# zgojcic/3D_multiview_reg

Measured on AMD Instinct MI355X. Metric: point-cloud pairs/s (feat+match+filter+SVD), 3DMatch 20k-pt, 1/2/4/8 GPU, higher is better.
Workload: dtype f32 (bf16x3 MFMA operands); 1 GPU; one synthetic 3DMatch-scale scene per GPU (configs[2]): 30 fragments x ~20393 voxels (0.025 m) -> FCGF -> rand 5000 samples -> soft feature-NN for all 435 pairs -> OANet (128ch, 500 clusters, 2 blocks) -> weighted Procrustes -> all-gather of (R,t,conf); sampler=rand, fragments_per_gpu=30, pairs_per_gpu=435, samples=5000, voxels_mean=20393, math=f32eq, oanet_point_layout=chunk-major, spconv_presplit_planes=False, spatial_map_order=False, library=2d143fd7778128e4, parallelism=dp1 (one scene per rank, RCCL all-gather of records)

## Files before the change

### 3d_multiview_reg_amd/csrc/knobs.hpp

```cpp
#pragma once

namespace mvr {

constexpr int GPU_CUS = 256;

extern int g_gemm_h;
extern int g_pconv_h;
extern int g_attn_h;
extern int g_spconv_h;
extern int g_feat_nn_fast;

enum ForcePath : int {
  FORCE_FEAT_NN_ONLINE = 0,
  FORCE_GENERIC_GEMM = 1,
  FORCE_UNFUSED_ATTN = 2,
  FORCE_NO_CONV1_FOLD = 3,
  FORCE_POOL_NOSPLIT = 4,
  FORCE_UNPOOL8 = 5,
  FORCE_ROW_LAYOUT = 6,
  FORCE_COUNT = 7
};
extern int g_force[FORCE_COUNT];

}
```

### 3d_multiview_reg_amd/csrc/spconv.hip

```cpp

#include "common.hpp"
#include "knobs.hpp"
#include "mfma_bf16.hpp"
#include "prof.hpp"
#include "sparse.hpp"

namespace mvr {

typedef float floatx16 __attribute__((ext_vector_type(16)));

struct SpArgs {
  const float* in; int64_t ldin; int Cin;
  const int32_t* nbr; int K; int64_t Mout;
  const int32_t* perm;
  const float* W; int Cout;
  const float* bias;
  mvr_bn_p bn; float bn_eps;
  const float* res; int64_t ldres;
  int relu;
  float* out; int64_t ldout;
  int* range; const int* guard; int epoch;
  const uint16_t* inp;
  uint16_t* outp;
};

constexpr int SP_KMAX = 32;
__device__ __attribute__((aligned(16))) float g_sp_zero[4];


#ifndef SP_TRACE
#define SP_TRACE 0
#endif
#if SP_TRACE
__device__ unsigned long long g_sp_trace[8];
#define SPSTAMP(slot)                                                  \
  do {                                                                 \
    unsigned long long t_;                                             \
    __builtin_amdgcn_sched_barrier(0);                                 \
    asm volatile("s_memtime %0\n\ts_waitcnt lgkmcnt(0)" : "=s"(t_));  \
    __builtin_amdgcn_sched_barrier(0);                                 \
    tr[prev_slot] += t_ - t_last;                                      \
    t_last = t_;                                                       \
    prev_slot = (slot);                                                \
  } while (0)
#else
#define SPSTAMP(slot) do {} while (0)
#endif

constexpr int SB_K = 32;
constexpr int SB_BST = 40;
constexpr int SB_CP = 128;
#ifndef SPBX_WBUF
#define SPBX_WBUF 1
#endif
#ifndef SPBX_NS32
#define SPBX_NS32 3
#endif
#ifndef SPBX_NS64
#define SPBX_NS64 3
#endif
#ifndef SPBX_NS128
#define SPBX_NS128 3
#endif
#ifndef SPBX_PS_NS32
#define SPBX_PS_NS32 3
#endif
#ifndef SPBX_PS_NS64
#define SPBX_PS_NS64 3
#endif
#ifndef SPBX_PS_NS128
#define SPBX_PS_NS128 2
#endif

template <int TN, int NS, int H, int PS>
__global__ __launch_bounds__(256, 2) void spconv_bx_kernel(SpArgs a, const uint16_t* __restrict__ wimg, int64_t CoutP,
                                                           const float* __restrict__ isc) {
  using namespace bx;
  constexpr int NPL = planes<H>();
  constexpr float XS = H ? 64.f : 1.f;
  constexpr int TM = 128;
  constexpr int NJ = TN / 32;
  constexpr int BPL = TN * SB_BST;
  constexpr int BG = NPL * BPL * 2 / 16;
  constexpr int GPT = (BG + 255) / 256;
  if (a.guard && *a.guard != a.epoch) return;
  __shared__ __attribute__((aligned(16))) uint16_t Bs[2][NPL * BPL];
  __shared__ int32_t nb[TM][SP_KMAX + 1];
  __shared__ int klist[SP_KMAX];
  __shared__ int orow_s[TM];
  __shared__ unsigned wmask[4];

  const int tid = threadIdx.x, lane = tid & 63, w = tid >> 6;
  const int l32 = lane & 31, h = lane >> 5;
#if SP_TRACE
  unsigned long long tr[8] = {0, 0, 0, 0, 0, 0, 0, 0}, t_last = __builtin_amdgcn_s_memtime();
  int prev_slot = 0;
#endif
  const int gy = (a.Cout + TN - 1) / TN;
  const int64_t t = (int64_t)blockIdx.x;
  const int64_t o0 = (t / gy) * TM;
  const int c0 = (int)(t % gy) * TN;
  const int K = a.K;

  if (tid < TM) {
    const int64_t o = o0 + tid;
    orow_s[tid] = o < a.Mout ? (int)(a.perm ? a.perm[o] : o) : -1;
  }
  __syncthreads();
  {
    constexpr int EMAX = (TM * SP_KMAX + 255) / 256;
    const int dq = 256 / K, dr = 256 - dq * K;
    int row = tid / K, k = tid - row * K;
    int vv[EMAX], ks[EMAX], rs[EMAX];
#pragma unroll
    for (int i = 0; i < EMAX; ++i) {
      ks[i] = k;
      rs[i] = row;
      vv[i] = -1;
      if (row < TM) {
        const int orow = orow_s[row];
        if (orow >= 0) vv[i] = a.nbr ? a.nbr[(int64_t)orow * K + k] : orow;
      }
      row += dq;
      k += dr;
      if (k >= K) {
        k -= K;
        ++row;
      }
    }
    unsigned m = 0;
#pragma unroll
    for (int i = 0; i < EMAX; ++i) {
      if (rs[i] < TM) {
        nb[rs[i]][ks[i]] = vv[i];
        if (vv[i] >= 0) m |= 1u << ks[i];
      }
    }
#pragma unroll
    for (int off = 32; off > 0; off >>= 1) m |= (unsigned)__shfl_xor((int)m, off, 64);
    if (lane == 0) wmask[w] = m;
  }
  __syncthreads();
  const unsigned kmask = wmask[0] | wmask[1] | wmask[2] | wmask[3];
  if (tid < K && ((kmask >> tid) & 1u)) klist[__popc(kmask & ((1u << tid) - 1u))] = tid;
  const int nk = __popc(kmask);
  __syncthreads();

  const int nci = (a.Cin + SB_K - 1) / SB_K;
  const int steps = nk * nci;
  const int row = 32 * w + l32;

  typedef float f32x4 __attribute__((ext_vector_type(4)));
  static_assert(!(PS && H), "pre-split planes are split-bf16");
  struct ASet {
    float4 v[PS ? 1 : 4];
    bf16x8 pv[PS ? 2 : 1][PS ? 3 : 1];
    f32x4 bq[GPT];
  };
  auto load_a = [&](int s, ASet& A) {
    if (s >= steps) s = steps - 1;
    const int k = klist[s / nci];
    const int ci0 = (s % nci) * SB_K;
    const int src = nb[row][k];
    if (PS) {
      const uint16_t* base = a.inp + (int64_t)(src >= 0 ? src : 0) * 3 * a.ldin;
#pragma unroll
      for (int st = 0; st < 2; ++st)
#pragma unroll
        for (int pl = 0; pl < 3; ++pl) {
          const uint16_t* pq = base + pl * a.ldin + ci0 + 16 * st + 8 * h;
          A.pv[st % (PS ? 2 : 1)][pl % (PS ? 3 : 1)] =
              *reinterpret_cast<const bf16x8*>(src >= 0 ? (const void*)pq : (const void*)g_sp_zero);
        }
    } else {
      const float* base = a.in + (int64_t)(src >= 0 ? src : 0) * a.ldin;
#pragma unroll
      for (int q = 0; q < 4; ++q) {
        const int ci = ci0 + 16 * (q >> 1) + 8 * h + 4 * (q & 1);
        const float* pq = src >= 0 ? base + ci : g_sp_zero;
        A.v[q % (PS ? 1 : 4)] = *reinterpret_cast<const float4*>(pq);
      }
    }
    const int cb = s % nci;
    const char* wb = reinterpret_cast<const char*>(wimg) + ((int64_t)(k * nci + cb) * NPL * CoutP + c0) * SB_BST * 2;
#if SPBX_WBUF
    const __amdgpu_buffer_rsrc_t rw = __builtin_amdgcn_make_buffer_rsrc(const_cast<char*>(wb), (short)0, 0x7fffffff,
                                                                        0x00020000);
#pragma unroll
    for (int i = 0; i < GPT; ++i) {
      const int g = min(tid + 256 * i, BG - 1);
      const int pl = g / (TN * 5), wi = g - pl * (TN * 5);
      A.bq[i] = __builtin_bit_cast(f32x4, __builtin_amdgcn_raw_buffer_load_b128(
                                              rw, pl * (int)CoutP * SB_BST * 2 + wi * 16, 0, 0));
    }
#else
#pragma unroll
    for (int i = 0; i < GPT; ++i) {
      const int g = min(tid + 256 * i, BG - 1);
      const int pl = g / (TN * 5), wi = g - pl * (TN * 5);
      A.bq[i] = *reinterpret_cast<const f32x4*>(wb + (int64_t)pl * CoutP * SB_BST * 2 + wi * 16);
    }
#endif
  };
  bool xbad = false;
  float xmx = 0.f;
  auto frag_a = [&](const ASet& A, int st) {
    if (PS) {
      FragT<H> f;
#pragma unroll
      for (int pl = 0; pl < planes<H>(); ++pl)
        f.p[pl] = __builtin_bit_cast(typename FragT<H>::V, A.pv[st % (PS ? 2 : 1)][pl % (PS ? 3 : 1)]);
      return f;
    }
    float v[8];
    const float4 x0 = A.v[(2 * st) % (PS ? 1 : 4)], x1 = A.v[(2 * st + 1) % (PS ? 1 : 4)];
    v[0] = x0.x; v[1] = x0.y; v[2] = x0.z; v[3] = x0.w;
    v[4] = x1.x; v[5] = x1.y; v[6] = x1.z; v[7] = x1.w;
    if (H) {
      float mx = 0.f;
#pragma unroll
      for (int i = 0; i < 8; ++i) {
        v[i] *= XS;
        mx = fmaxf(mx, fabsf(v[i]));
      }
      xbad |= !(mx < F16_RANGE);
      xmx = fmaxf(xmx, mx);
    }
    return split8t<H>(v);
  };
  auto store_b = [&](const ASet& A, int buf) {
    char* dst = reinterpret_cast<char*>(Bs[buf]);
#pragma unroll
    for (int i = 0; i < GPT; ++i) {
      const int g = tid + 256 * i;
      if (g < BG) *reinterpret_cast<f32x4*>(dst + g * 16) = A.bq[i];
    }
  };

  floatx16 acc[NJ];
#pragma unroll
  for (int j = 0; j < NJ; ++j)
#pragma unroll
    for (int r = 0; r < 16; ++r) acc[j][r] = 0.f;

  if (steps > 0) {
    ASet A[NS];
    SPSTAMP(7);
#pragma unroll
    for (int u = 0; u < NS; ++u) load_a(u, A[u]);
    store_b(A[0], 0);
    __syncthreads();
    auto step = [&](int s, ASet& A, const ASet& An) {
      const int cur = s & 1;
      SPSTAMP(1);
      if (s + 1 < steps) store_b(An, cur ^ 1);
      SPSTAMP(2);
      const FragT<H> fa0 = frag_a(A, 0), fa1 = frag_a(A, 1);
      SPSTAMP(3);
      load_a(s + NS, A);
      SPSTAMP(4);
      const uint16_t* Bq = Bs[cur];
#pragma unroll
      for (int st = 0; st < 2; ++st) {
        const FragT<H>& fa = st ? fa1 : fa0;
#pragma unroll
        for (int j = 0; j < NJ; ++j) {
          const uint16_t* bp = Bq + (32 * j + l32) * SB_BST + 16 * st + 8 * h;
          const FragT<H> fb = ld_frag<H>(reinterpret_cast<const char*>(bp), 2 * BPL);
          acc[j] = mma<H>(fa, fb, acc[j]);
        }
      }
      SPSTAMP(5);
      __syncthreads();
    };
    int s = 0;
    for (; s + NS - 1 < steps; s += NS) {
#pragma unroll
      for (int u = 0; u < NS; ++u) step(s + u, A[u], A[(u + 1) % NS]);
    }
#pragma unroll
    for (int u = 0; u < NS - 1; ++u)
      if (s + u < steps) step(s + u, A[u], A[(u + 1) % NS]);
  }

  SPSTAMP(6);
  int orr[16];
#pragma unroll
  for (int r = 0; r < 16; ++r) orr[r] = orow_s[32 * w + (r & 3) + 8 * (r >> 2) + 4 * h];
#pragma unroll
  for (int j = 0; j < NJ; ++j) {
    const int c = c0 + j * 32 + l32;
    if (c >= a.Cout) continue;
    float bsc = 1.f, bsh = 0.f;
    if (a.bn.gamma) {
      bsc = a.bn.gamma[c] / sqrtf(a.bn.var[c] + a.bn_eps);
      bsh = a.bn.beta[c] - a.bn.mean[c] * bsc;
    }
    const float bias = a.bias ? a.bias[c] : 0.f;
    const float is = H ? isc[c] : 1.f;
    float rv[16];
#pragma unroll
    for (int r = 0; r < 16; ++r) rv[r] = a.res && orr[r] >= 0 ? a.res[(int64_t)orr[r] * a.ldres + c] : 0.f;
#pragma unroll
    for (int r = 0; r < 16; ++r) {
      if (orr[r] < 0) continue;
      float v = (H ? acc[j][r] * is : acc[j][r]) + bias;
      v = fmaf(v, bsc, bsh);
      if (a.res) v += rv[r];
      if (a.relu) v = fmaxf(v, 0.f);
      a.out[(int64_t)orr[r] * a.ldout + c] = v;
      if (a.outp) bx::store_planes(a.outp + (int64_t)orr[r] * 3 * a.ldout + c, a.ldout, v);
    }
  }
  if (H && __any(xbad || (xmx > 0.f && xmx < 0.125f)) && lane == 0) atomicExch(a.range, a.epoch);
#if SP_TRACE
  SPSTAMP(0);
  if (lane == 0)
// ... 40 lines not shown
  uint16_t* row = img + ((kb * 3) * CoutP + c) * SB_BST + 8 * q;
  *reinterpret_cast<bf16x8*>(row) = f.h;
  *reinterpret_cast<bf16x8*>(row + CoutP * SB_BST) = f.m;
  *reinterpret_cast<bf16x8*>(row + 2 * CoutP * SB_BST) = f.l;
  const float sc = wsc[c];
#pragma unroll
  for (int i = 0; i < 8; ++i) v[i] *= sc;
  const FragT<1> g = split8t<1>(v);
  uint16_t* row16 = img16 + ((kb * 2) * CoutP + c) * SB_BST + 8 * q;
  *reinterpret_cast<f16x8*>(row16) = g.p[0];
  *reinterpret_cast<f16x8*>(row16 + CoutP * SB_BST) = g.p[1];
}

#ifndef SPCONV_MATH_DEFAULT
#define SPCONV_MATH_DEFAULT 0
#endif
int g_spconv_h = SPCONV_MATH_DEFAULT;

}

using namespace mvr;

static int64_t sp_coutp(int Cout) { return ((int64_t)Cout + SB_CP - 1) / SB_CP * SB_CP; }

static size_t sp_bf16_bytes(int K, int Cin, int Cout) {
  return (size_t)K * ((Cin + SB_K - 1) / SB_K) * 3 * sp_coutp(Cout) * SB_BST * 2;
}
static size_t sp_f16_bytes(int K, int Cin, int Cout) { return sp_bf16_bytes(K, Cin, Cout) / 3 * 2; }

extern "C" size_t mvr_spconv_wimage_bytes(int K, int Cin, int Cout) {
  if (K <= 0 || Cin <= 0 || Cout <= 0) return 0;
  return sp_bf16_bytes(K, Cin, Cout) + sp_f16_bytes(K, Cin, Cout) + 2 * sp_coutp(Cout) * sizeof(float);
}

extern "C" int mvr_spconv_wimage(const float* W, int K, int Cin, int Cout, void* img, size_t bytes, hipStream_t s) {
  if (!W || !img || K <= 0 || K > SP_KMAX || Cin <= 0 || Cout <= 0 || bytes < mvr_spconv_wimage_bytes(K, Cin, Cout) ||
      (reinterpret_cast<uintptr_t>(img) & 15))
    return MVR_EINVAL;
  const int nci = (Cin + SB_K - 1) / SB_K;
  const int64_t CoutP = sp_coutp(Cout);
  const int64_t total = (int64_t)K * nci * CoutP * 4;
  char* base = reinterpret_cast<char*>(img);
  uint16_t* img16 = reinterpret_cast<uint16_t*>(base + sp_bf16_bytes(K, Cin, Cout));
  float* wsc = reinterpret_cast<float*>(base + sp_bf16_bytes(K, Cin, Cout) + sp_f16_bytes(K, Cin, Cout));
  hipLaunchKernelGGL(spconv_wscale_kernel, dim3((unsigned)((CoutP * 64 + 255) / 256)), dim3(256), 0, s, W, K, Cin, Cout,
                     CoutP, wsc, wsc + CoutP);
  MVR_CHECK_LAUNCH();
  hipLaunchKernelGGL(spconv_wimage_kernel, dim3((unsigned)((total + 255) / 256)), dim3(256), 0, s, W, K, Cin, Cout, nci,
                     CoutP, reinterpret_cast<uint16_t*>(img), img16, wsc);
  MVR_CHECK_LAUNCH();
  return MVR_OK;
}

extern "C" int mvr_spconv_x(const float* in, int64_t ldin, int Cin, const int32_t* nbr, const int32_t* perm, int K,
                            int64_t Mout, const float* W, int Cout, const float* bias, mvr_bn_p bn, float bn_eps,
                            const float* res, int64_t ldres, int relu, float* out, int64_t ldout, const void* wimg,
                            int32_t* range_flag, const uint16_t* in_planes, uint16_t* out_planes, hipStream_t s) {
  if (Cin <= 0 || Cout <= 0 || K <= 0 || K > SP_KMAX || Mout < 0) return MVR_EINVAL;
  if (Mout == 0) return MVR_OK;
  if (!in || !W || !out || !wimg) return MVR_EINVAL;
  if ((in_planes && ((ldin & 7) || (reinterpret_cast<uintptr_t>(in_planes) & 15))) ||
      (out_planes && (reinterpret_cast<uintptr_t>(out_planes) & 1)))
    return MVR_EINVAL;
  if (reinterpret_cast<uintptr_t>(wimg) & 15) return MVR_EINVAL;
  if (!nbr && K != 1) return MVR_EINVAL;
  if ((Cin % SB_K) || (Cout & 3) || (ldin & 3) || (reinterpret_cast<uintptr_t>(in) & 15) ||
      (reinterpret_cast<uintptr_t>(W) & 15))
    return MVR_EINVAL;
  SpArgs a{in, ldin, Cin, nbr, K, Mout, perm, W, Cout, bias, bn, bn_eps, res, ldres, relu, out, ldout,
           nullptr, nullptr, 0, in_planes, out_planes};
  ProfScope prof(PK_SPCONV, 2.0 * Mout * (double)K * Cin * Cout,
                 (double)Mout * (Cin + Cout) * 4.0 + (nbr ? (double)Mout * K * 4.0 : 0.0) + 4.0 * K * Cin * Cout, s);
  const char* base = reinterpret_cast<const char*>(wimg);
  const uint16_t* wi = reinterpret_cast<const uint16_t*>(wimg);
  const uint16_t* wi16 = reinterpret_cast<const uint16_t*>(base + sp_bf16_bytes(K, Cin, Cout));
  const int64_t CoutP = sp_coutp(Cout);
  const float* isc = reinterpret_cast<const float*>(base + sp_bf16_bytes(K, Cin, Cout) + sp_f16_bytes(K, Cin, Cout)) +
                     CoutP;
  const unsigned gx = (unsigned)((Mout + 127) / 128);
  const bool h1 = g_spconv_h && range_flag && Cout > 64 && res != out;
  if (h1) {
    if (hipMemsetAsync(range_flag, 0, sizeof(int32_t), s) != hipSuccess) return MVR_ELAUNCH;
    a.range = range_flag;
    a.epoch = 1;
  }
#define MVR_SPL(TN_, NS_, PNS_, GY)                                                                             \
  do {                                                                                                         \
    if (h1) {                                                                                                  \
      hipLaunchKernelGGL((spconv_bx_kernel<TN_, NS_, 1, 0>), dim3(gx * (GY)), dim3(256), 0, s, a, wi16, CoutP, isc); \
      MVR_CHECK_LAUNCH();                                                                                      \
      a.guard = a.range;                                                                                       \
      a.range = nullptr;                                                                                       \
    }                                                                                                          \
    if (in_planes)                                                                                             \
      hipLaunchKernelGGL((spconv_bx_kernel<TN_, PNS_, 0, 1>), dim3(gx * (GY)), dim3(256), 0, s, a, wi, CoutP, isc); \
    else                                                                                                       \
      hipLaunchKernelGGL((spconv_bx_kernel<TN_, NS_, 0, 0>), dim3(gx * (GY)), dim3(256), 0, s, a, wi, CoutP, isc); \
  } while (0)
  if (Cout <= 32)
    MVR_SPL(32, SPBX_NS32, SPBX_PS_NS32, 1);
  else if (Cout <= 64)
    MVR_SPL(64, SPBX_NS64, SPBX_PS_NS64, (Cout + 63) / 64);
  else
    MVR_SPL(128, SPBX_NS128, SPBX_PS_NS128, (Cout + 127) / 128);
#undef MVR_SPL
  MVR_CHECK_LAUNCH();
  return MVR_OK;
}

extern "C" int mvr_spconv(const float* in, int64_t ldin, int Cin, const int32_t* nbr, const int32_t* perm, int K,
                          int64_t Mout, const float* W, int Cout, const float* bias, mvr_bn_p bn, float bn_eps,
                          const float* res, int64_t ldres, int relu, float* out, int64_t ldout, const void* wimg,
                          int32_t* range_flag, hipStream_t s) {
  return mvr_spconv_x(in, ldin, Cin, nbr, perm, K, Mout, W, Cout, bias, bn, bn_eps, res, ldres, relu, out, ldout, wimg,
                      range_flag, nullptr, nullptr, s);
}

#if SP_TRACE
extern "C" int mvr_spconv_trace(unsigned long long* out, int reset) {
  if (hipMemcpyFromSymbol(out, HIP_SYMBOL(mvr::g_sp_trace), sizeof(unsigned long long) * 8) != hipSuccess) return -1;
  if (reset) {
    unsigned long long z[8] = {0, 0, 0, 0, 0, 0, 0, 0};
    if (hipMemcpyToSymbol(HIP_SYMBOL(mvr::g_sp_trace), z, sizeof(z)) != hipSuccess) return -1;
  }
  return 0;
}
#endif
```

### 3d_multiview_reg_amd/lib/_native.py

```python
import ctypes
import os

import torch

_PKG = os.path.dirname(os.path.dirname(os.path.abspath(__file__)))
LIB_PATH = os.environ.get("MVR_LIB") or os.path.join(_PKG, "libmvreg_hip.so")
_lib = None

c_i64 = ctypes.c_int64
c_int = ctypes.c_int
c_float = ctypes.c_float
c_vp = ctypes.c_void_p
c_size = ctypes.c_size_t


class ConvP(ctypes.Structure):
    _fields_ = [("weight", c_vp), ("bias", c_vp)]


class BnP(ctypes.Structure):
    _fields_ = [("gamma", c_vp), ("beta", c_vp), ("mean", c_vp), ("var", c_vp)]


class PointCNP(ctypes.Structure):
# ... 72 lines not shown
    "mvr_radius_index_bytes": (c_size, [c_i64]),
    "mvr_radius_index_build": (c_int, [c_vp, c_vp, c_int, c_i64, ctypes.c_double, c_vp, c_size, c_vp]),
    "mvr_radius_overlap_count": (c_int, [c_vp, c_size, c_vp, c_vp, c_int, c_i64, c_vp, c_vp, c_int, c_i64,
                                         ctypes.c_double, c_vp, c_vp]),
    "mvr_icp_refine": (c_int, [c_vp, c_size, c_vp, c_vp, c_int, c_i64, ctypes.c_double, c_vp, c_vp, c_int,
                               ctypes.c_double, c_int, ctypes.c_double, ctypes.c_double, c_vp, c_vp, c_vp, c_vp, c_vp,
                               c_vp, c_vp, c_vp]),
    "mvr_estimate_normals": (c_int, [c_vp, c_size, c_vp, c_vp, c_int, c_i64, ctypes.c_double, ctypes.c_double, c_vp,
                                     c_vp, c_vp, c_vp]),
    "mvr_icp_refine_plane": (c_int, [c_vp, c_size, c_vp, c_vp, c_vp, c_int, c_i64, ctypes.c_double, c_vp, c_vp, c_int,
                                     ctypes.c_double, c_int, ctypes.c_double, ctypes.c_double, c_vp, c_vp, c_vp, c_vp,
                                     c_vp, c_vp, c_vp, c_vp]),
    "mvr_icp_refine_generalized": (c_int, [c_vp, c_size, c_vp, c_vp, c_vp, c_int, c_i64, ctypes.c_double, c_vp, c_vp,
                                           c_int, ctypes.c_double, ctypes.c_double, c_int, ctypes.c_double,
                                           ctypes.c_double, c_vp, c_vp, c_vp, c_vp, c_vp, c_vp, c_vp, c_vp]),
    "mvr_pair_information": (c_int, [c_vp, c_size, c_vp, c_vp, c_int, c_i64, ctypes.c_double, c_vp, c_vp, c_int,
                                     ctypes.c_double, c_vp, c_vp, c_vp, c_vp, c_vp]),
    "mvr_compute_fpfh_workspace_bytes": (c_size, [c_i64]),
    "mvr_compute_fpfh": (c_int, [c_vp, c_size, c_vp, c_vp, c_vp, c_int, c_i64, ctypes.c_double, ctypes.c_double, c_vp,
                                 c_vp, c_vp, c_size, c_vp]),
    "mvr_feat_match": (c_int, [c_vp, c_int, c_vp, c_int, c_i64, c_vp, c_vp, c_int, c_i64, c_i64, c_vp, c_vp, c_vp]),
    "mvr_posegraph_workspace_bytes": (c_size, [c_int, c_int, c_int]),
    "mvr_posegraph_optimize": (c_int, [c_vp, c_vp, c_vp, c_vp, c_vp, c_i64, c_vp, c_vp, c_int, c_int, c_int, c_int,
                                       c_vp, c_vp, c_int, ctypes.c_double, ctypes.c_double, ctypes.c_double, c_vp,
                                       c_vp, c_i64, c_vp, c_vp, c_vp, c_vp, c_vp, c_vp, c_size, c_vp]),
    "mvr_fuse_scene_workspace_bytes": (c_size, [c_i64]),
    "mvr_fuse_scene": (c_int, [c_vp, c_vp, c_vp, c_int, c_i64, c_vp, c_vp, ctypes.c_double, c_vp, c_size, c_vp, c_vp,
                               c_vp, c_vp, c_vp, c_vp]),
    "mvr_hash_table_bytes": (c_size, [c_i64]),
    "mvr_voxelize_workspace_bytes": (c_size, [c_i64]),
    "mvr_voxelize_hint_workspace_bytes": (c_size, [c_i64, c_i64]),
    "mvr_voxelize_hint": (c_int, [c_vp, c_vp, c_int, c_i64, ctypes.c_double, c_i64, c_vp, c_size, c_vp, c_vp, c_vp,
                                  c_vp]),
    "mvr_voxelize": (c_int, [c_vp, c_vp, c_int, c_i64, ctypes.c_double, c_vp, c_size, c_vp, c_vp, c_vp, c_vp]),
    "mvr_voxelize_f64": (c_int, [c_vp, c_vp, c_int, c_i64, ctypes.c_double, c_vp, c_size, c_vp, c_vp, c_vp, c_vp]),
    "mvr_coords_downsample_workspace_bytes": (c_size, [c_i64]),
    "mvr_coords_downsample": (c_int, [c_vp, c_i64, c_int, c_int, c_vp, c_size, c_vp, c_vp, c_vp]),
    "mvr_hash_build": (c_int, [c_vp, c_i64, c_vp, c_size, c_vp]),
    "mvr_hash_build_lattice": (c_int, [c_vp, c_i64, c_int, c_vp, c_size, c_vp]),
    "mvr_kernel_map": (c_int, [c_vp, c_i64, c_vp, c_size, c_int, c_int, c_int, c_vp, c_vp]),
    "mvr_kernel_map_x": (c_int, [c_vp, c_i64, c_vp, c_size, c_int, c_int, c_int, c_vp, c_vp, c_vp]),
    "mvr_kernel_map_sym": (c_int, [c_vp, c_i64, c_vp, c_size, c_int, c_vp, c_vp]),
    "mvr_kernel_map_transpose": (c_int, [c_vp, c_i64, c_int, c_vp, c_i64, c_vp]),
    "mvr_kernel_map_order_bytes": (c_size, [c_i64]),
    "mvr_kernel_map_order": (c_int, [c_vp, c_vp, c_int, c_i64, c_int, c_vp, c_vp, c_size, c_vp]),
    "mvr_kernel_map_orders_bytes": (c_size, [c_i64]),
    "mvr_kernel_map_orders": (c_int, [c_int, c_vp, c_vp, c_vp, c_vp, c_int, c_vp, c_vp, c_size, c_vp]),
    "mvr_radix_sort_pairs_bytes": (c_size, [c_i64]),
    "mvr_radix_sort_pairs": (c_int, [c_vp, c_vp, c_i64, c_int, c_vp, c_vp, c_size, c_vp]),
    "mvr_spconv": (c_int, [c_vp, c_i64, c_int, c_vp, c_vp, c_int, c_i64, c_vp, c_int, c_vp, BnP, c_float, c_vp, c_i64,
                           c_int, c_vp, c_i64, c_vp, c_vp, c_vp]),
    "mvr_spconv_x": (c_int, [c_vp, c_i64, c_int, c_vp, c_vp, c_int, c_i64, c_vp, c_int, c_vp, BnP, c_float, c_vp,
                             c_i64, c_int, c_vp, c_i64, c_vp, c_vp, c_vp, c_vp, c_vp]),
    "mvr_spconv_c1_x": (c_int, [c_vp, c_i64, c_vp, c_i64, c_size, c_vp, c_int, c_int, c_vp, c_int, BnP, c_float,
                                c_int, c_vp, c_i64, c_vp, c_vp]),
    "mvr_spconv_wimage_bytes": (c_size, [c_int, c_int, c_int]),
    "mvr_spconv_wimage": (c_int, [c_vp, c_int, c_int, c_int, c_vp, c_size, c_vp]),
    "mvr_brick_map_bytes": (c_size, [c_i64]),
    "mvr_brick_map_build": (c_int, [c_vp, c_i64, c_vp, c_size, c_vp]),
    "mvr_brick_map_build_stride": (c_int, [c_vp, c_i64, c_int, c_vp, c_size, c_vp]),
    "mvr_spconv_c1": (c_int, [c_vp, c_i64, c_vp, c_i64, c_size, c_vp, c_int, c_int, c_vp, c_int, BnP, c_float, c_int,
                              c_vp, c_i64, c_vp]),
    "mvr_l2norm_rows": (c_int, [c_vp, c_i64, c_int, c_i64, c_vp]),
    "mvr_prof_set": (c_int, [c_int]),
    "mvr_prof_mask": (c_int, [ctypes.c_uint]),
    "mvr_prof_seq": (c_int, [c_vp, c_vp, c_int]),
    "mvr_prof_get": (c_int, [c_int, ctypes.POINTER(ctypes.c_double), ctypes.POINTER(ctypes.c_longlong),
                             ctypes.POINTER(ctypes.c_double), ctypes.POINTER(ctypes.c_double)]),
    "mvr_oan_last_layout": (c_int, []),
    "mvr_source_hash": (c_int, [ctypes.c_char_p, c_size]),
    "mvr_xs_to_channels": (c_int, [c_vp, c_i64, c_i64, c_int, c_int, c_int, c_vp, c_i64, c_i64, c_vp]),
}

EXPORTS = tuple(_SIGS)


def lib():
    global _lib
    if _lib is None:
        if not os.path.exists(LIB_PATH):
            raise RuntimeError("libmvreg_hip.so not found at %s — run __graft_entry__.build() "
                               "(there is no CPU fallback for the HIP path)" % LIB_PATH)
        L = ctypes.CDLL(LIB_PATH)
        for name, (res, args) in _SIGS.items():
            f = getattr(L, name)
            f.restype = res
            f.argtypes = args
        _lib = L
    return _lib


_hip_ok = False


def require_hip(t=None):
    global _hip_ok
    if not _hip_ok:
        if not torch.cuda.is_available():
            raise RuntimeError("mvreg HIP path: no HIP device available (no CPU fallback)")
        _hip_ok = True
    if t is not None and t.device.type != "cuda":
        raise RuntimeError("mvreg HIP path: tensor on %s, expected a HIP device" % t.device)


def stream():
    return c_vp(torch.cuda.current_stream().cuda_stream)
# ... 1 lines not shown

def ptr(t):
    if t is None:
        return None
    return c_vp(t.data_ptr())


def check(rc, name):
    if rc != 0:
        raise RuntimeError("%s failed with code %d" % (name, rc))


def source_hash():
    buf = ctypes.create_string_buffer(128)
    check(lib().mvr_source_hash(buf, len(buf)), "mvr_source_hash")
    return buf.value.decode()


PROF_KINDS = {"conv_pts": 0, "embed": 1, "pool": 2, "unpool": 3, "oafilter": 4, "small": 5, "procrustes": 6,
              "feat_nn": 7, "spconv": 8, "sparse_misc": 9, "pointcn": 10}
RANSAC_CHECKED_PROF = {"check": 11, "scan": 12, "eval": 13, "select": 14}


def prof_set(on):
    check(lib().mvr_prof_set(int(on)), "mvr_prof_set")


def prof_mask(kinds=None):
    m = 0xFFFFFFFF if kinds is None else sum(1 << (PROF_KINDS[k] if isinstance(k, str) else int(k)) for k in kinds)
    check(lib().mvr_prof_mask(m), "mvr_prof_mask")


def prof_seq():
    import numpy as np
    L = lib()
    n = L.mvr_prof_seq(None, None, 0)
    k = np.zeros(max(n, 1), np.int32)
    b = np.zeros(max(n, 1), np.float64)
    L.mvr_prof_seq(k.ctypes.data, b.ctypes.data, n)
    names = {v: s for s, v in PROF_KINDS.items()}
    return [(names.get(int(k[i]), str(int(k[i]))), float(b[i])) for i in range(n)]


def prof_get(kind):
    ms, n, fl, by = ctypes.c_double(), ctypes.c_longlong(), ctypes.c_double(), ctypes.c_double()
    k = PROF_KINDS[kind] if isinstance(kind, str) else int(kind)
    check(lib().mvr_prof_get(k, ctypes.byref(ms), ctypes.byref(n), ctypes.byref(fl), ctypes.byref(by)),
          "mvr_prof_get")
    return ms.value, n.value, fl.value, by.value


MATH_KERNELS = "pconv_math,attn_math,spconv_math,gemm_f16,feat_nn"
FORCE = {"feat_nn_online": 0, "generic_gemm": 1, "unfused_attn": 2, "no_conv1_fold": 3, "pool_nosplit": 4,
         "unpool8": 5, "row_layout": 6}


def math_state():
    L = lib()
    m = L.mvr_set_math(0)
    L.mvr_set_math(m)
    return m


def set_math(mode):
    L = lib()
    L.mvr_set_math({"f32eq": 0, "split16": 1}[mode])
    m = math_state()
    dtype = "f32 (bf16x3 MFMA operands)" if not m else "mixed: split-fp16 (22-bit) operands in " + MATH_KERNELS
    return {"mode": "split16" if m else "f32eq", "dtype": dtype, "knobs": {"split16": m}}


class force:

    def __init__(self, what, value=1):
        self.what, self.value = FORCE[what], int(value)

    def __enter__(self):
        self.prev = lib().mvr_debug_force(self.what, self.value)
        return self

    def __exit__(self, *a):
        lib().mvr_debug_force(self.what, self.prev)


_ws_cache = {}
_flag_cache = {}


def flag_word(device=None):
    idx = (device.index if device is not None and device.index is not None else torch.cuda.current_device())
    key = (idx, torch.cuda.current_stream(idx).cuda_stream)
    buf = _flag_cache.get(key)
    if buf is None:
        buf = torch.zeros(64, dtype=torch.int32, device=torch.device("cuda", idx))
        _flag_cache[key] = buf
    return buf


def workspace(nbytes, device):
    idx = device.index if device.index is not None else torch.cuda.current_device()
    key = (idx, torch.cuda.current_stream(idx).cuda_stream)
    buf = _ws_cache.get(key)
    if buf is None or buf.numel() < nbytes:
        buf = torch.empty(max(int(nbytes), 1), dtype=torch.uint8, device=device)
        _ws_cache[key] = buf
    if _WS_POISON:
        buf[:int(nbytes)].fill_(0x7F)
# ... 5 lines not shown
```

### 3d_multiview_reg_amd/lib/descriptor/fcgf.py

```python
import os

import torch
import torch.nn as nn

from lib import _native as N
from lib.sparse import SparseTensor


CONV1_BRICKS = os.environ.get("MVR_CONV1_BRICKS", "1") == "1"
PRESPLIT = os.environ.get("MVR_SPCONV_PRESPLIT", "0") == "1"


def _planes(M, ld, dev):
    return torch.empty(M, 3, ld, dtype=torch.int16, device=dev) if PRESPLIT else None


class _MEConv(nn.Module):

    def __init__(self, cin, cout, ksize, has_bias=False):
        super().__init__()
        self.kernel_size = ksize
        self.kernel = nn.Parameter(torch.empty(ksize ** 3, cin, cout))
        nn.init.kaiming_normal_(self.kernel.data.view(-1, cout), nonlinearity="relu")
        self.bias = nn.Parameter(torch.zeros(1, cout)) if has_bias else None
# ... 30 lines not shown
        self.norm2 = _MENorm(planes, bn_momentum)


def _bn(norm):
    if norm is None:
        return N.BnP(None, None, None, None), 1e-5
    b = norm.bn
    return N.BnP(b.weight.data_ptr(), b.bias.data_ptr(), b.running_mean.data_ptr(), b.running_var.data_ptr()), b.eps


class FCGFNet(nn.Module):
    NORM_TYPE = "BN"
    BLOCK_NORM_TYPE = "BN"
    CHANNELS = [None, 32, 64, 128, 256]
    TR_CHANNELS = [None, 64, 64, 64, 128]

    def __init__(self, in_channels=1, out_channels=32, bn_momentum=0.05, normalize_feature=True,
                 conv1_kernel_size=7, D=3):
        super().__init__()
        C, T = self.CHANNELS, self.TR_CHANNELS
        self.D = D
        self.normalize_feature = normalize_feature
        self.conv1_kernel_size = conv1_kernel_size
        self.conv1 = _MEConv(in_channels, C[1], conv1_kernel_size)
        self.norm1 = _MENorm(C[1], bn_momentum)
        self.block1 = BasicBlockBN(C[1], C[1], bn_momentum)
        self.conv2 = _MEConv(C[1], C[2], 3)
        self.norm2 = _MENorm(C[2], bn_momentum)
        self.block2 = BasicBlockBN(C[2], C[2], bn_momentum)
        self.conv3 = _MEConv(C[2], C[3], 3)
        self.norm3 = _MENorm(C[3], bn_momentum)
        self.block3 = BasicBlockBN(C[3], C[3], bn_momentum)
        self.conv4 = _MEConv(C[3], C[4], 3)
        self.norm4 = _MENorm(C[4], bn_momentum)
        self.block4 = BasicBlockBN(C[4], C[4], bn_momentum)
        self.conv4_tr = _MEConv(C[4], T[4], 3)
        self.norm4_tr = _MENorm(T[4], bn_momentum)
        self.block4_tr = BasicBlockBN(T[4], T[4], bn_momentum)
        self.conv3_tr = _MEConv(C[3] + T[4], T[3], 3)
        self.norm3_tr = _MENorm(T[3], bn_momentum)
        self.block3_tr = BasicBlockBN(T[3], T[3], bn_momentum)
        self.conv2_tr = _MEConv(C[2] + T[3], T[2], 3)
        self.norm2_tr = _MENorm(T[2], bn_momentum)
        self.block2_tr = BasicBlockBN(T[2], T[2], bn_momentum)
        self.conv1_tr = _MEConv(C[1] + T[2], T[1], 1)
        self.final = _MEConv(T[1], out_channels, 1, has_bias=True)

    def _conv(self, x, ldx, conv, km, M, out, ldout, norm=None, res=None, ldres=0, relu=False, bias=None, xp=None,
              outp=None):
        bnp, eps = _bn(norm)
        K, cin, cout = conv.kernel.shape
        nbr, perm = km if km is not None else (None, None)
        wimg = conv.wimage()
        N.check(N.lib().mvr_spconv_x(N.ptr(x), ldx, cin, N.ptr(nbr), N.ptr(perm), K, M, N.ptr(conv.kernel), cout,
                                     N.ptr(bias), bnp, eps, N.ptr(res), ldres, int(relu), N.ptr(out), ldout,
                                     N.ptr(wimg), N.ptr(N.flag_word(x.device)), N.ptr(xp), N.ptr(outp), N.stream()),
                "mvr_spconv_x")
        return out

    def _block(self, blk, x, ldx, km, M, out, ldout, xp=None, outp=None):
        c = blk.conv1.kernel.shape[2]
        t = torch.empty(M, c, device=x.device)
        tp = _planes(M, c, x.device)
        self._conv(x, ldx, blk.conv1, km, M, t, c, blk.norm1, relu=True, xp=xp, outp=tp)
        self._conv(t, c, blk.conv2, km, M, out, ldout, blk.norm2, res=x, ldres=ldx, relu=True, xp=tp, outp=outp)
        return out

    def forward(self, x):
        N.require_hip()
        f32 = torch.float32
        if not all(t.is_cuda and t.dtype is f32 and t.is_contiguous()
                   for t in (*self.parameters(), *self.buffers()) if t.dtype.is_floating_point):
            raise RuntimeError("FCGFNet parameters must be contiguous float32 on a HIP device")
        if self.training:
            raise NotImplementedError("FCGFNet on the HIP path runs in eval mode (BatchNorm running statistics)")
        cm = x.coords_man
        cm.prepare_orders()

        def km(kind, s):
            return cm.kernel_map(kind, s), cm.kernel_map_order(kind, s)
        dev = x.F.device
        C, T = self.CHANNELS, self.TR_CHANNELS
        M = [cm.coords_at(s).shape[0] for s in (1, 2, 4, 8)]
        L = N.lib()
        feat = x.F.float().contiguous()
        if feat.shape[1] != 1:
            raise NotImplementedError("conv1 kernel supports in_channels=1 (all reference configs)")
        s1 = torch.empty(M[0], C[1], device=dev)
        bnp, eps = _bn(self.norm1)
        bricks = cm.brick_map(1)
        oc = None if (self.conv1_kernel_size == 7 and CONV1_BRICKS) else N.ptr(cm.coords_at(1))
        s1p = _planes(M[0], C[1], dev) if oc is None else None
        N.check(L.mvr_spconv_c1_x(oc, M[0], N.ptr(bricks), M[0], bricks.numel(), N.ptr(feat),
                                  self.conv1_kernel_size, 1, N.ptr(self.conv1.kernel), C[1], bnp, eps, 0, N.ptr(s1),
                                  C[1], N.ptr(s1p), N.stream()), "mvr_spconv_c1_x")
        cat1 = torch.empty(M[0], T[2] + C[1], device=dev)
        cat2 = torch.empty(M[1], T[3] + C[2], device=dev)
        cat3 = torch.empty(M[2], T[4] + C[3], device=dev)
        w1, w2, w3 = cat1.shape[1], cat2.shape[1], cat3.shape[1]
        cat1p, cat2p, cat3p = (_planes(M[i], w, dev) for i, w in ((0, w1), (1, w2), (2, w3)))
        skip1, skip2, skip3 = cat1[:, T[2]:], cat2[:, T[3]:], cat3[:, T[4]:]

        def sl(p, c0):
            return p[:, :, c0:] if p is not None else None
        skip1p, skip2p, skip3p = sl(cat1p, T[2]), sl(cat2p, T[3]), sl(cat3p, T[4])
        self._block(self.block1, s1, C[1], km("s1", 1), M[0], skip1, w1, s1p, skip1p)
        t2 = torch.empty(M[1], C[2], device=dev)
        t2p = _planes(M[1], C[2], dev)
        self._conv(skip1, w1, self.conv2, km("down", 1), M[1], t2, C[2], self.norm2, xp=skip1p, outp=t2p)
        self._block(self.block2, t2, C[2], km("s1", 2), M[1], skip2, w2, t2p, skip2p)
# ... 32 lines not shown
```

### include/mvreg.h

```cpp
#ifndef MVREG_H
#define MVREG_H
#include <stddef.h>
#include <stdint.h>

#ifdef __cplusplus
extern "C" {
#endif

typedef struct ihipStream_t* mvr_stream_t;

#define MVR_OK 0
#define MVR_EINVAL -1
#define MVR_ELAUNCH -2

int mvr_procrustes(const float* x1, const float* x2, int64_t x_pstride, int64_t x_nstride, float* w,
                   int64_t w_pstride, const int32_t* guard_pos, float* w_copy, int64_t wc_pstride, int P, int N,
                   int normalize, float eps, float* R, float* t, float* res, int64_t res_pstride, float* res_copy,
                   int64_t rc_pstride, int32_t* status, int guard_group, mvr_stream_t stream);
int mvr_procrustes_f64(const double* x1, const double* x2, int64_t x_pstride, int64_t x_nstride, double* w,
                       int64_t w_pstride, const int32_t* guard_pos, double* w_copy, int64_t wc_pstride, int P, int N,
                       int normalize, double eps, double* R, double* t, double* res, int64_t res_pstride,
                       double* res_copy, int64_t rc_pstride, int32_t* status, int guard_group,
                       mvr_stream_t stream);

// ... 172 lines not shown
int mvr_feat_nn_gumbel(const float* Fq, int64_t fq_fstride, const float* Ft, int64_t ft_fstride, const float* Xq,
                       int64_t xq_fstride, const float* Xt, int64_t xt_fstride, const int64_t* pairs, int P, int Nq,
                       int Mt, int C, float inv_tau, int hard, uint64_t seed, float* out, int64_t out_pstride,
                       int64_t out_nstride, int32_t* idx_out, mvr_stream_t stream);

int mvr_feat_knn2(const float* Fq, int64_t fq_fstride, const float* Ft, int64_t ft_fstride, const int64_t* pairs,
                  int P, int Nq, int Mt, int C, int32_t* idx2_out, double* dist2_out, mvr_stream_t stream);

int mvr_gather_rows(const float* src, int C, const int64_t* idx, int n, float* dst, mvr_stream_t stream);

size_t mvr_hash_table_bytes(int64_t M);
size_t mvr_voxelize_workspace_bytes(int64_t n);
int mvr_voxelize(const float* xyz, const int64_t* frag_off, int B, int64_t n, double voxel, void* workspace,
                 size_t workspace_bytes, int32_t* coords_out, int64_t* sel_out, int64_t* counts_out,
                 mvr_stream_t stream);
int mvr_voxelize_f64(const double* xyz, const int64_t* frag_off, int B, int64_t n, double voxel, void* workspace,
                     size_t workspace_bytes, int32_t* coords_out, int64_t* sel_out, int64_t* counts_out,
                     mvr_stream_t stream);
size_t mvr_voxelize_hint_workspace_bytes(int64_t n, int64_t distinct_hint);
int mvr_voxelize_hint(const float* xyz, const int64_t* frag_off, int B, int64_t n, double voxel,
                      int64_t distinct_hint, void* ws, size_t ws_bytes, int32_t* coords_out, int64_t* sel_out,
                      int64_t* counts_out, mvr_stream_t stream);
size_t mvr_coords_downsample_workspace_bytes(int64_t M);
int mvr_coords_downsample(const int32_t* coords, int64_t M, int B, int stride_out, void* workspace,
                          size_t workspace_bytes, int32_t* coords_out, int64_t* counts_out, mvr_stream_t stream);
int mvr_hash_build(const int32_t* coords, int64_t M, void* table, size_t table_bytes, mvr_stream_t stream);
int mvr_hash_build_lattice(const int32_t* coords, int64_t M, int stride, void* table, size_t table_bytes,
                           mvr_stream_t stream);
int mvr_kernel_map(const int32_t* out_coords, int64_t Mout, const void* in_table, size_t in_table_bytes, int ksize,
                   int step, int transposed, int32_t* nbr, mvr_stream_t stream);
int mvr_kernel_map_x(const int32_t* out_coords, int64_t Mout, const void* in_table, size_t in_table_bytes, int ksize,
                     int step, int transposed, int32_t* nbr, const int32_t* row_order, mvr_stream_t stream);
int mvr_kernel_map_sym(const int32_t* coords, int64_t M, const void* table, size_t table_bytes, int step, int32_t* nbr,
                       mvr_stream_t stream);
int mvr_kernel_map_transpose(const int32_t* src, int64_t Ms, int K, int32_t* dst, int64_t Md, mvr_stream_t stream);
size_t mvr_kernel_map_order_bytes(int64_t Mout);
int mvr_kernel_map_order(const int32_t* nbr, const int32_t* out_coords, int step, int64_t Mout, int K, int32_t* perm,
                         void* workspace, size_t workspace_bytes, mvr_stream_t stream);
size_t mvr_kernel_map_orders_bytes(int64_t total);
int mvr_kernel_map_orders(int n_maps, const int32_t* const* nbr, const int32_t* const* out_coords, const int* steps,
                          const int64_t* Mo, int K, int32_t* perm_out, void* workspace, size_t workspace_bytes,
                          mvr_stream_t stream);
size_t mvr_radix_sort_pairs_bytes(int64_t n);
int mvr_radix_sort_pairs(const uint64_t* keys, const int32_t* vals, int64_t n, int bits, int32_t* vals_out,
                         void* workspace, size_t workspace_bytes, mvr_stream_t stream);
int mvr_spconv(const float* in, int64_t ldin, int Cin, const int32_t* nbr, const int32_t* perm, int K, int64_t Mout,
               const float* W, int Cout, const float* bias, mvr_bn_p bn, float bn_eps, const float* res,
               int64_t ldres, int relu, float* out, int64_t ldout, const void* wimg, int32_t* range_flag,
               mvr_stream_t stream);
int mvr_spconv_x(const float* in, int64_t ldin, int Cin, const int32_t* nbr, const int32_t* perm, int K, int64_t Mout,
                 const float* W, int Cout, const float* bias, mvr_bn_p bn, float bn_eps, const float* res,
                 int64_t ldres, int relu, float* out, int64_t ldout, const void* wimg, int32_t* range_flag,
                 const uint16_t* in_planes, uint16_t* out_planes, mvr_stream_t stream);
size_t mvr_spconv_wimage_bytes(int K, int Cin, int Cout);
int mvr_spconv_wimage(const float* W, int K, int Cin, int Cout, void* img, size_t bytes, mvr_stream_t stream);
size_t mvr_brick_map_bytes(int64_t M);
int mvr_brick_map_build(const int32_t* coords, int64_t M, void* workspace, size_t workspace_bytes,
                        mvr_stream_t stream);
int mvr_brick_map_build_stride(const int32_t* coords, int64_t M, int stride, void* workspace, size_t workspace_bytes,
                               mvr_stream_t stream);
int mvr_spconv_c1(const int32_t* out_coords, int64_t Mout, const void* in_bricks, int64_t Min, size_t in_bricks_bytes,
                  const float* feat, int ksize, int step, const float* W, int Cout, mvr_bn_p bn, float bn_eps,
                  int relu, float* out, int64_t ldout, mvr_stream_t stream);
int mvr_spconv_c1_x(const int32_t* out_coords, int64_t Mout, const void* in_bricks, int64_t Min,
                    size_t in_bricks_bytes, const float* feat, int ksize, int step, const float* W, int Cout,
                    mvr_bn_p bn, float bn_eps, int relu, float* out, int64_t ldout, uint16_t* out_planes,
                    mvr_stream_t stream);
int mvr_l2norm_rows(float* x, int64_t M, int C, int64_t ld, mvr_stream_t stream);

int mvr_sample_rand_mt19937(uint32_t* key, int32_t* pos, const int64_t* counts, int B, int tgt, int64_t* out,
                            int64_t* ws);

int mvr_prof_set(int on);
int mvr_prof_mask(unsigned mask);
int mvr_prof_get(int kind, double* ms, long long* launches, double* flops, double* bytes);
int mvr_prof_seq(int* kinds, double* bytes, int cap);
int mvr_source_hash(char* buf, size_t cap);

#ifdef __cplusplus
}
#endif
#endif
```

Before: 10620 pairs/s.

## Use 32-bit buffer-resource loads with precomputed byte offsets in sparse conv

Adds a sparse-conv kernel variant that stores each neighbour index as a premultiplied byte offset, with INT_MIN marking a missing neighbour. Input and weight-image gathers go through AMD buffer resource loads, which return zero for out-of-range offsets, so the 64-bit address arithmetic and the per-step zero-pointer select are no longer needed. The active-kernel list is walked with an incremental bitmask iterator, which drops the klist shared-memory build and one block barrier. The variant is chosen only when the input row count is passed and the tensor sizes fit in 31-bit offsets. It adds a new entry point and a force flag that falls back to the old path.

```diff
diff --git a/3d_multiview_reg_amd/csrc/knobs.hpp b/3d_multiview_reg_amd/csrc/knobs.hpp
--- a/3d_multiview_reg_amd/csrc/knobs.hpp
+++ b/3d_multiview_reg_amd/csrc/knobs.hpp
@@ -18,7 +18,8 @@
   FORCE_POOL_NOSPLIT = 4,
   FORCE_UNPOOL8 = 5,
   FORCE_ROW_LAYOUT = 6,
-  FORCE_COUNT = 7
+  FORCE_SPCONV_ADDR64 = 7,
+  FORCE_COUNT = 8
 };
 extern int g_force[FORCE_COUNT];
 
diff --git a/3d_multiview_reg_amd/csrc/spconv.hip b/3d_multiview_reg_amd/csrc/spconv.hip
--- a/3d_multiview_reg_amd/csrc/spconv.hip
+++ b/3d_multiview_reg_amd/csrc/spconv.hip
@@ -1,3 +1,5 @@
+
+#include <climits>
 
 #include "common.hpp"
 #include "knobs.hpp"
@@ -22,6 +24,7 @@
   int* range; const int* guard; int epoch;
   const uint16_t* inp;
   uint16_t* outp;
+  uint32_t in_bytes;
 };
 
 constexpr int SP_KMAX = 32;
@@ -53,6 +56,9 @@
 #ifndef SPBX_WBUF
 #define SPBX_WBUF 1
 #endif
+#ifndef SPBX_GBUF
+#define SPBX_GBUF 1
+#endif
 #ifndef SPBX_NS32
 #define SPBX_NS32 3
 #endif
@@ -72,7 +78,7 @@
 #define SPBX_PS_NS128 2
 #endif
 
-template <int TN, int NS, int H, int PS>
+template <int TN, int NS, int H, int PS, int BO>
 __global__ __launch_bounds__(256, 2) void spconv_bx_kernel(SpArgs a, const uint16_t* __restrict__ wimg, int64_t CoutP,
                                                            const float* __restrict__ isc) {
   using namespace bx;
@@ -128,10 +134,12 @@
         ++row;
       }
     }
+    const int rowb = (int)a.ldin * (PS ? 6 : 4);
     unsigned m = 0;
 #pragma unroll
     for (int i = 0; i < EMAX; ++i) {
       if (rs[i] < TM) {
+        if (BO) vv[i] = vv[i] >= 0 ? vv[i] * rowb : INT_MIN;
         nb[rs[i]][ks[i]] = vv[i];
         if (vv[i] >= 0) m |= 1u << ks[i];
       }
@@ -141,10 +149,14 @@
     if (lane == 0) wmask[w] = m;
   }
   __syncthreads();
-  const unsigned kmask = wmask[0] | wmask[1] | wmask[2] | wmask[3];
-  if (tid < K && ((kmask >> tid) & 1u)) klist[__popc(kmask & ((1u << tid) - 1u))] = tid;
+  unsigned kmask = wmask[0] | wmask[1] | wmask[2] | wmask[3];
+  if (BO) {
+    kmask = (unsigned)__builtin_amdgcn_readfirstlane((int)kmask);
+  } else {
+    if (tid < K && ((kmask >> tid) & 1u)) klist[__popc(kmask & ((1u << tid) - 1u))] = tid;
+  }
   const int nk = __popc(kmask);
-  __syncthreads();
+  if (!BO) __syncthreads();
 
   const int nci = (a.Cin + SB_K - 1) / SB_K;
   const int steps = nk * nci;
@@ -157,7 +169,52 @@
     bf16x8 pv[PS ? 2 : 1][PS ? 3 : 1];
     f32x4 bq[GPT];
   };
-  auto load_a = [&](int s, ASet& A) {
+  unsigned lrem = kmask;
+  int lk = kmask ? __builtin_ctz(kmask) : 0, lcb = 0;
+  const int hb = (PS ? 16 : 32) * h;
+  const int wstep = NPL * (int)CoutP * SB_BST * 2;
+  const void* gbase = PS ? (const void*)a.inp : (const void*)a.in;
+  const __amdgpu_buffer_rsrc_t rin =
+      __builtin_amdgcn_make_buffer_rsrc(const_cast<void*>(gbase), (short)0, (int)a.in_bytes, 0x00020000);
+  const __amdgpu_buffer_rsrc_t rwi = __builtin_amdgcn_make_buffer_rsrc(
+      const_cast<char*>(reinterpret_cast<const char*>(wimg)) + (int64_t)c0 * SB_BST * 2, (short)0, 0x7fffffff,
+      0x00020000);
+  int woff[GPT];
+#pragma unroll
+  for (int i = 0; i < GPT; ++i) {
+    const int g = min(tid + 256 * i, BG - 1);
+    const int pl = g / (TN * 5), wi = g - pl * (TN * 5);
+    woff[i] = pl * (int)CoutP * SB_BST * 2 + wi * 16;
+  }
+  auto load_a = [&](int s, ASet& A, const FragT<H>* fa = nullptr) {
+    if (BO) {
+      int off = nb[row][lk];
+      if (!PS && fa) asm volatile("" : "+v"(off) : "v"(fa[0].p[NPL - 1]), "v"(fa[1].p[NPL - 1]));
+      const int vo = off + hb;
+      if (PS) {
+#pragma unroll
+        for (int st = 0; st < 2; ++st)
+#pragma unroll
+          for (int pl = 0; pl < 3; ++pl)
+            A.pv[st % (PS ? 2 : 1)][pl % (PS ? 3 : 1)] = __builtin_bit_cast(
+                bf16x8, __builtin_amdgcn_raw_buffer_load_b128(rin, vo + 32 * st, pl * (int)a.ldin * 2 + lcb * SB_K * 2, 0));
+      } else {
+#pragma unroll
+        for (int q = 0; q < 4; ++q)
+          A.v[q % (PS ? 1 : 4)] = __builtin_bit_cast(
+              float4, __builtin_amdgcn_raw_buffer_load_b128(rin, vo + 64 * (q >> 1) + 16 * (q & 1), lcb * SB_K * 4, 0));
+      }
+      const int ws = (lk * nci + lcb) * wstep;
+#pragma unroll
+      for (int i = 0; i < GPT; ++i)
+        A.bq[i] = __builtin_bit_cast(f32x4, __builtin_amdgcn_raw_buffer_load_b128(rwi, woff[i], ws, 0));
+      const unsigned nrem = lrem & (lrem - 1);
+      const bool inblk = lcb + 1 < nci, next = !inblk && nrem != 0;
+      lcb = inblk ? lcb + 1 : (next ? 0 : lcb);
+      lrem = next ? nrem : lrem;
+      lk = next ? __builtin_ctz(nrem) : lk;
+      return;
+    }
     if (s >= steps) s = steps - 1;
     const int k = klist[s / nci];
     const int ci0 = (s % nci) * SB_K;
@@ -255,14 +312,14 @@
       SPSTAMP(1);
       if (s + 1 < steps) store_b(An, cur ^ 1);
       SPSTAMP(2);
-      const FragT<H> fa0 = frag_a(A, 0), fa1 = frag_a(A, 1);
+      const FragT<H> faq[2] = {frag_a(A, 0), frag_a(A, 1)};
       SPSTAMP(3);
-      load_a(s + NS, A);
+      load_a(s + NS, A, faq);
       SPSTAMP(4);
       const uint16_t* Bq = Bs[cur];
 #pragma unroll
       for (int st = 0; st < 2; ++st) {
-        const FragT<H>& fa = st ? fa1 : fa0;
+        const FragT<H>& fa = faq[st];
 #pragma unroll
         for (int j = 0; j < NJ; ++j) {
           const uint16_t* bp = Bq + (32 * j + l32) * SB_BST + 16 * st + 8 * h;
@@ -409,10 +466,11 @@
   return MVR_OK;
 }
 
-extern "C" int mvr_spconv_x(const float* in, int64_t ldin, int Cin, const int32_t* nbr, const int32_t* perm, int K,
+extern "C" int mvr_spconv_n(const float* in, int64_t ldin, int Cin, const int32_t* nbr, const int32_t* perm, int K,
                             int64_t Mout, const float* W, int Cout, const float* bias, mvr_bn_p bn, float bn_eps,
                             const float* res, int64_t ldres, int relu, float* out, int64_t ldout, const void* wimg,
-                            int32_t* range_flag, const uint16_t* in_planes, uint16_t* out_planes, hipStream_t s) {
+                            int32_t* range_flag, const uint16_t* in_planes, uint16_t* out_planes, int64_t Min,
+                            hipStream_t s) {
   if (Cin <= 0 || Cout <= 0 || K <= 0 || K > SP_KMAX || Mout < 0) return MVR_EINVAL;
   if (Mout == 0) return MVR_OK;
   if (!in || !W || !out || !wimg) return MVR_EINVAL;
@@ -435,24 +493,37 @@
   const float* isc = reinterpret_cast<const float*>(base + sp_bf16_bytes(K, Cin, Cout) + sp_f16_bytes(K, Cin, Cout)) +
                      CoutP;
   const unsigned gx = (unsigned)((Mout + 127) / 128);
+  const bool bo = SPBX_GBUF && !g_force[FORCE_SPCONV_ADDR64] && Min >= (nbr ? 1 : Mout) && ldin >= Cin &&
+                  (double)Min * ldin * (in_planes ? 6 : 4) < 2147483648.0 &&
+                  sp_bf16_bytes(K, Cin, Cout) < (size_t)1 << 31;
+  const uint32_t inb = bo ? (uint32_t)(((Min - 1) * ldin + Cin) * 4) : 0;
+  const uint32_t inpb = bo ? (uint32_t)(((3 * Min - 1) * ldin + Cin) * 2) : 0;
   const bool h1 = g_spconv_h && range_flag && Cout > 64 && res != out;
   if (h1) {
     if (hipMemsetAsync(range_flag, 0, sizeof(int32_t), s) != hipSuccess) return MVR_ELAUNCH;
     a.range = range_flag;
     a.epoch = 1;
   }
-#define MVR_SPL(TN_, NS_, PNS_, GY)                                                                             \
-  do {                                                                                                         \
-    if (h1) {                                                                                                  \
-      hipLaunchKernelGGL((spconv_bx_kernel<TN_, NS_, 1, 0>), dim3(gx * (GY)), dim3(256), 0, s, a, wi16, CoutP, isc); \
-      MVR_CHECK_LAUNCH();                                                                                      \
-      a.guard = a.range;                                                                                       \
-      a.range = nullptr;                                                                                       \
-    }                                                                                                          \
-    if (in_planes)                                                                                             \
-      hipLaunchKernelGGL((spconv_bx_kernel<TN_, PNS_, 0, 1>), dim3(gx * (GY)), dim3(256), 0, s, a, wi, CoutP, isc); \
-    else                                                                                                       \
-      hipLaunchKernelGGL((spconv_bx_kernel<TN_, NS_, 0, 0>), dim3(gx * (GY)), dim3(256), 0, s, a, wi, CoutP, isc); \
+#define MVR_SPK(TN_, NS_, H_, PS_, GY, WI)                                                                            \
+  do {                                                                                                               \
+    a.in_bytes = (PS_) ? inpb : inb;                                                                                 \
+    if (bo)                                                                                                          \
+      hipLaunchKernelGGL((spconv_bx_kernel<TN_, NS_, H_, PS_, 1>), dim3(gx * (GY)), dim3(256), 0, s, a, WI, CoutP, isc); \
+    else                                                                                                             \
+      hipLaunchKernelGGL((spconv_bx_kernel<TN_, NS_, H_, PS_, 0>), dim3(gx * (GY)), dim3(256), 0, s, a, WI, CoutP, isc); \
+  } while (0)
+#define MVR_SPL(TN_, NS_, PNS_, GY)          \
+  do {                                       \
+    if (h1) {                                \
+      MVR_SPK(TN_, NS_, 1, 0, GY, wi16);     \
+      MVR_CHECK_LAUNCH();                    \
+      a.guard = a.range;                     \
+      a.range = nullptr;                     \
+    }                                        \
+    if (in_planes)                           \
+      MVR_SPK(TN_, PNS_, 0, 1, GY, wi);      \
+    else                                     \
+      MVR_SPK(TN_, NS_, 0, 0, GY, wi);       \
   } while (0)
   if (Cout <= 32)
     MVR_SPL(32, SPBX_NS32, SPBX_PS_NS32, 1);
@@ -461,8 +532,17 @@
   else
     MVR_SPL(128, SPBX_NS128, SPBX_PS_NS128, (Cout + 127) / 128);
 #undef MVR_SPL
+#undef MVR_SPK
   MVR_CHECK_LAUNCH();
   return MVR_OK;
+}
+
+extern "C" int mvr_spconv_x(const float* in, int64_t ldin, int Cin, const int32_t* nbr, const int32_t* perm, int K,
+                            int64_t Mout, const float* W, int Cout, const float* bias, mvr_bn_p bn, float bn_eps,
+                            const float* res, int64_t ldres, int relu, float* out, int64_t ldout, const void* wimg,
+                            int32_t* range_flag, const uint16_t* in_planes, uint16_t* out_planes, hipStream_t s) {
+  return mvr_spconv_n(in, ldin, Cin, nbr, perm, K, Mout, W, Cout, bias, bn, bn_eps, res, ldres, relu, out, ldout, wimg,
+                      range_flag, in_planes, out_planes, -1, s);
 }
 
 extern "C" int mvr_spconv(const float* in, int64_t ldin, int Cin, const int32_t* nbr, const int32_t* perm, int K,
diff --git a/3d_multiview_reg_amd/lib/_native.py b/3d_multiview_reg_amd/lib/_native.py
--- a/3d_multiview_reg_amd/lib/_native.py
+++ b/3d_multiview_reg_amd/lib/_native.py
@@ -148,6 +148,8 @@
                            c_int, c_vp, c_i64, c_vp, c_vp, c_vp]),
     "mvr_spconv_x": (c_int, [c_vp, c_i64, c_int, c_vp, c_vp, c_int, c_i64, c_vp, c_int, c_vp, BnP, c_float, c_vp,
                              c_i64, c_int, c_vp, c_i64, c_vp, c_vp, c_vp, c_vp, c_vp]),
+    "mvr_spconv_n": (c_int, [c_vp, c_i64, c_int, c_vp, c_vp, c_int, c_i64, c_vp, c_int, c_vp, BnP, c_float, c_vp,
+                             c_i64, c_int, c_vp, c_i64, c_vp, c_vp, c_vp, c_vp, c_i64, c_vp]),
     "mvr_spconv_c1_x": (c_int, [c_vp, c_i64, c_vp, c_i64, c_size, c_vp, c_int, c_int, c_vp, c_int, BnP, c_float,
                                 c_int, c_vp, c_i64, c_vp, c_vp]),
     "mvr_spconv_wimage_bytes": (c_size, [c_int, c_int, c_int]),
@@ -255,7 +257,7 @@
 
 MATH_KERNELS = "pconv_math,attn_math,spconv_math,gemm_f16,feat_nn"
 FORCE = {"feat_nn_online": 0, "generic_gemm": 1, "unfused_attn": 2, "no_conv1_fold": 3, "pool_nosplit": 4,
-         "unpool8": 5, "row_layout": 6}
+         "unpool8": 5, "row_layout": 6, "spconv_addr64": 7}
 
 
 def math_state():
diff --git a/3d_multiview_reg_amd/lib/descriptor/fcgf.py b/3d_multiview_reg_amd/lib/descriptor/fcgf.py
--- a/3d_multiview_reg_amd/lib/descriptor/fcgf.py
+++ b/3d_multiview_reg_amd/lib/descriptor/fcgf.py
@@ -106,10 +106,11 @@
         K, cin, cout = conv.kernel.shape
         nbr, perm = km if km is not None else (None, None)
         wimg = conv.wimage()
-        N.check(N.lib().mvr_spconv_x(N.ptr(x), ldx, cin, N.ptr(nbr), N.ptr(perm), K, M, N.ptr(conv.kernel), cout,
+        N.check(N.lib().mvr_spconv_n(N.ptr(x), ldx, cin, N.ptr(nbr), N.ptr(perm), K, M, N.ptr(conv.kernel), cout,
                                      N.ptr(bias), bnp, eps, N.ptr(res), ldres, int(relu), N.ptr(out), ldout,
-                                     N.ptr(wimg), N.ptr(N.flag_word(x.device)), N.ptr(xp), N.ptr(outp), N.stream()),
-                "mvr_spconv_x")
+                                     N.ptr(wimg), N.ptr(N.flag_word(x.device)), N.ptr(xp), N.ptr(outp), x.shape[0],
+                                     N.stream()),
+                "mvr_spconv_n")
         return out
 
     def _block(self, blk, x, ldx, km, M, out, ldout, xp=None, outp=None):
diff --git a/include/mvreg.h b/include/mvreg.h
--- a/include/mvreg.h
+++ b/include/mvreg.h
@@ -248,6 +248,10 @@
                  const float* W, int Cout, const float* bias, mvr_bn_p bn, float bn_eps, const float* res,
                  int64_t ldres, int relu, float* out, int64_t ldout, const void* wimg, int32_t* range_flag,
                  const uint16_t* in_planes, uint16_t* out_planes, mvr_stream_t stream);
+int mvr_spconv_n(const float* in, int64_t ldin, int Cin, const int32_t* nbr, const int32_t* perm, int K, int64_t Mout,
+                 const float* W, int Cout, const float* bias, mvr_bn_p bn, float bn_eps, const float* res,
+                 int64_t ldres, int relu, float* out, int64_t ldout, const void* wimg, int32_t* range_flag,
+                 const uint16_t* in_planes, uint16_t* out_planes, int64_t rows_in, mvr_stream_t stream);
 size_t mvr_spconv_wimage_bytes(int K, int Cin, int Cout);
 int mvr_spconv_wimage(const float* W, int K, int Cin, int Cout, void* img, size_t bytes, mvr_stream_t stream);
 size_t mvr_brick_map_bytes(int64_t M);
```

Result: no change. 10640 pairs/s, median of 6 (+0.3%).
